# ZAX130/SmileCode

Measured on AMD Instinct MI355X. Metric: volume-pairs/sec (160x192x160) fwd+bwd, higher is better.
Workload: dtype f32; 1 GPU; ModeT 160x192x160 fp32, batch=1/GPU, full train step NCC+Grad3d fwd+bwd+Adam-amsgrad; global_batch=1, parallelism=dp1, allreduce=one flat all-reduce after backward

## Files before the change

### smilecode_amd/csrc/na.hip

```cpp
#include "common.h"
#include "drpb_reduce.h"
#include <cstdlib>

namespace {

constexpr int HD = 6;
constexpr int TZ = 4, TY = 4, TX = 16;
constexpr int HZ = TZ + 2, HY = TY + 2, HX = TX + 2;
constexpr int HVOX = HZ * HY * HX;
constexpr int NTHREADS = TZ * TY * TX;

struct TileGeom {
  int tiles_x, tiles_y, tiles_z;
};

__device__ __forceinline__ void tile_origin(int tile, const TileGeom g, int& z0, int& y0, int& x0) {
  const int tx = tile % g.tiles_x;
  const int t2 = tile / g.tiles_x;
  x0 = tx * TX;
  y0 = (t2 % g.tiles_y) * TY;
  z0 = (t2 / g.tiles_y) * TZ;
}

constexpr int KT_IT = (HVOX * 3 + NTHREADS - 1) / NTHREADS;
__device__ __forceinline__ float2 bf2_unpack(unsigned u) { return make_float2(__uint_as_float(u << 16), __uint_as_float(u & 0xffff0000u)); }
template <bool QK16 = false>
__device__ __forceinline__ void stage_k_load(float2 (&r)[KT_IT], const float* __restrict__ k, int64_t bbase, int z0, int y0,
                                             int x0, int D, int H, int W, int C, int hoff) {
  bool inside[KT_IT];
#pragma unroll
  for (int j = 0; j < KT_IT; ++j) {
    const int idx = min((int)threadIdx.x + j * NTHREADS, HVOX * 3 - 1);
    const int v = idx / 3, part = idx - v * 3;
    const int hx = v % HX, t = v / HX;
    const int hy = t % HY, hz = t / HY;
    const int z = z0 + hz - 1, y = y0 + hy - 1, x = x0 + hx - 1;
    const bool in = z >= 0 && z < D && y >= 0 && y < H && x >= 0 && x < W;
    const int64_t off = (bbase + (in ? ((int64_t)z * H + y) * W + x : 0)) * C + hoff + part * 2;
    if constexpr (QK16) r[j] = bf2_unpack(reinterpret_cast<const unsigned*>(k)[off >> 1]);
    else r[j] = *reinterpret_cast<const float2*>(k + off);
    inside[j] = in;
  }
#pragma unroll
  for (int j = 0; j < KT_IT; ++j) asm volatile("" : "+v"(r[j].x), "+v"(r[j].y));
#pragma unroll
  for (int j = 0; j < KT_IT; ++j)
    if (!inside[j]) r[j] = make_float2(0.f, 0.f);
}
__device__ __forceinline__ void stage_k_store(float* __restrict__ kt, const float2 (&r)[KT_IT]) {
#pragma unroll
  for (int j = 0; j < KT_IT; ++j) {
    const int idx = threadIdx.x + j * NTHREADS;
    if (idx < HVOX * 3) *reinterpret_cast<float2*>(kt + idx * 2) = r[j];
  }
}
template <bool QK16 = false>
__device__ __forceinline__ void stage_k_tile(float* __restrict__ kt, const float* __restrict__ k, int64_t bbase,
                                             int z0, int y0, int x0, int D, int H, int W, int C, int hoff) {
  float2 r[KT_IT];
  stage_k_load<QK16>(r, k, bbase, z0, y0, x0, D, H, W, C, hoff);
  stage_k_store(kt, r);
}

__device__ __forceinline__ void load6(const float* __restrict__ p, float (&r)[HD]) {
  const float2 a = *reinterpret_cast<const float2*>(p);
  const float2 b = *reinterpret_cast<const float2*>(p + 2);
  const float2 c = *reinterpret_cast<const float2*>(p + 4);
  r[0] = a.x; r[1] = a.y; r[2] = b.x; r[3] = b.y; r[4] = c.x; r[5] = c.y;
}

template <bool QK16>
__device__ __forceinline__ void load6g(const float* __restrict__ base, int64_t el, float (&r)[HD]) {
  if constexpr (QK16) {
    const unsigned* p = reinterpret_cast<const unsigned*>(base) + (el >> 1);
    const float2 a = bf2_unpack(p[0]), b = bf2_unpack(p[1]), c = bf2_unpack(p[2]);
    r[0] = a.x; r[1] = a.y; r[2] = b.x; r[3] = b.y; r[4] = c.x; r[5] = c.y;
  } else {
    load6(base + el, r);
  }
}

__device__ __forceinline__ void logits27(const float* __restrict__ kt, int lt, const float (&qs)[HD],
                                         const float* __restrict__ rpb_h, float (&lg)[27]) {
#pragma unroll
  for (int ki = 0; ki < 3; ++ki)
#pragma unroll
    for (int kj = 0; kj < 3; ++kj)
#pragma unroll
      for (int kk = 0; kk < 3; ++kk) {
        const int t = ki * 9 + kj * 3 + kk;
        float kv[HD];
        load6(kt + (lt + (ki * HY + kj) * HX + kk) * HD, kv);
        float s = rpb_h[t];
#pragma unroll
        for (int c = 0; c < HD; ++c) s = fmaf(qs[c], kv[c], s);
        lg[t] = s;
      }
}

__device__ __forceinline__ float softmax27(float (&lg)[27], float& m) {
  m = lg[0];
#pragma unroll
  for (int t = 1; t < 27; ++t) m = fmaxf(m, lg[t]);
  float s = 0.f;
#pragma unroll
  for (int t = 0; t < 27; ++t) {
    lg[t] = __expf(lg[t] - m);
    s += lg[t];
  }
  return 1.f / s;
}

template <bool QK16>
__global__ __launch_bounds__(NTHREADS) void na_fwd_kernel(const float* __restrict__ q, const float* __restrict__ k,
                                                          const float* __restrict__ rpb, float* __restrict__ out,
                                                          float* __restrict__ lse, int D, int H, int W, int heads,
                                                          float scale, TileGeom g) {
  __shared__ __attribute__((aligned(16))) float kt[HVOX * HD];
  __shared__ float rp[27];
  const int h = blockIdx.y, b = blockIdx.z;
  const int C = heads * HD;
  const int64_t V = (int64_t)D * H * W;
  int z0, y0, x0;
  tile_origin(blockIdx.x, g, z0, y0, x0);
  if (threadIdx.x < 27) rp[threadIdx.x] = rpb[h * 27 + threadIdx.x];
  stage_k_tile<QK16>(kt, k, (int64_t)b * V, z0, y0, x0, D, H, W, C, h * HD);
  __syncthreads();

  const int tx = threadIdx.x % TX, ty = (threadIdx.x / TX) % TY, tz = threadIdx.x / (TX * TY);
  const int z = z0 + tz, y = y0 + ty, x = x0 + tx;
  if (z >= D || y >= H || x >= W) return;
  const int64_t n = (int64_t)b * V + ((int64_t)z * H + y) * W + x;
  float qs[HD];
  load6g<QK16>(q, n * C + h * HD, qs);
#pragma unroll
  for (int c = 0; c < HD; ++c) qs[c] *= scale;
  float p[27];
  logits27(kt, (tz * HY + ty) * HX + tx, qs, rp, p);
  float mx;
  const float inv = softmax27(p, mx);
  if (lse) lse[n * heads + h] = mx - __logf(inv);
  float o0 = 0.f, o1 = 0.f, o2 = 0.f;
#pragma unroll
  for (int ki = 0; ki < 3; ++ki)
#pragma unroll
    for (int kj = 0; kj < 3; ++kj)
#pragma unroll
      for (int kk = 0; kk < 3; ++kk) {
        const float pv = p[ki * 9 + kj * 3 + kk];
        o0 += pv * (float)(ki - 1);
        o1 += pv * (float)(kj - 1);
        o2 += pv * (float)(kk - 1);
      }
  float* o = out + n * (heads * 3) + h * 3;
  o[0] = o0 * inv; o[1] = o1 * inv; o[2] = o2 * inv;
}

template <int N>
__device__ __forceinline__ void rs_step(float (&v)[32], int lane) {
  const bool up = (lane & N) != 0;
#pragma unroll
  for (int i = 0; i < N / 2; ++i) {
    const float keep = up ? v[i + N / 2] : v[i];
    const float send = up ? v[i] : v[i + N / 2];
    v[i] = keep + __shfl_xor(send, N, 64);
  }
}
__device__ __forceinline__ float wave_reduce_scatter32(const float (&v27)[27], int lane) {
  float v[32];
#pragma unroll
  for (int i = 0; i < 32; ++i) v[i] = i < 27 ? v27[i] : 0.f;
  rs_step<32>(v, lane); rs_step<16>(v, lane); rs_step<8>(v, lane); rs_step<4>(v, lane); rs_step<2>(v, lane);
  return v[0] + __shfl_xor(v[0], 1, 64);
}

constexpr int AUX = 5;

template <bool QK16>
__global__ __launch_bounds__(NTHREADS) void na_bwd_kernel(const float* __restrict__ q, const float* __restrict__ k,
                                                          const float* __restrict__ rpb, const float* __restrict__ out,
                                                          const float* __restrict__ lse, const float* __restrict__ dout,
                                                          float* __restrict__ dq, float* __restrict__ dk,
                                                          float* __restrict__ drpb_part, int D, int H, int W, int heads,
                                                          float scale, TileGeom g) {
  __shared__ __attribute__((aligned(16))) float kt[HVOX * HD];
  __shared__ __attribute__((aligned(16))) float qt[HVOX * HD];
  __shared__ float ax[HVOX * AUX];
  __shared__ float red[27 * (NTHREADS / 64)];
  __shared__ float rp[27];
  const int h = blockIdx.y, b = blockIdx.z;
  const int C = heads * HD;
  const int64_t V = (int64_t)D * H * W;
  int z0, y0, x0;
  tile_origin(blockIdx.x, g, z0, y0, x0);
  if (threadIdx.x < 27) rp[threadIdx.x] = rpb[h * 27 + threadIdx.x];
#ifdef NA_BWD_LDS_PAD
  __shared__ float lds_pad[NA_BWD_LDS_PAD];
  if (g.tiles_x < 0) { lds_pad[threadIdx.x % NA_BWD_LDS_PAD] = scale; __syncthreads(); rp[0] += lds_pad[(threadIdx.x * 7 + 1) % NA_BWD_LDS_PAD]; }
#endif
#ifdef NA_BWD_VGPR_CLOBBER
#define NA_STR2(x) #x
#define NA_STR(x) NA_STR2(x)
  asm volatile("" ::: "v" NA_STR(NA_BWD_VGPR_CLOBBER));
#endif
  {
    constexpr int AX_IT = (HVOX + NTHREADS - 1) / NTHREADS;
    float2 rk[KT_IT], rq[KT_IT];
    float ra[AX_IT][7];
    bool ain[AX_IT];
    stage_k_load<QK16>(rk, k, (int64_t)b * V, z0, y0, x0, D, H, W, C, h * HD);
    stage_k_load<QK16>(rq, q, (int64_t)b * V, z0, y0, x0, D, H, W, C, h * HD);
#pragma unroll
    for (int j = 0; j < AX_IT; ++j) {
      const int v = min((int)threadIdx.x + j * NTHREADS, HVOX - 1);
      const int hx = v % HX, t = v / HX;
      const int hy = t % HY, hz = t / HY;
      const int z = z0 + hz - 1, y = y0 + hy - 1, x = x0 + hx - 1;
      const bool in = z >= 0 && z < D && y >= 0 && y < H && x >= 0 && x < W;
      const int64_t n = (int64_t)b * V + (in ? ((int64_t)z * H + y) * W + x : 0);
      const float* go = dout + n * (heads * 3) + h * 3;
      const float* oo = out + n * (heads * 3) + h * 3;
      ra[j][0] = go[0]; ra[j][1] = go[1]; ra[j][2] = go[2];
      ra[j][3] = oo[0]; ra[j][4] = oo[1]; ra[j][5] = oo[2];
      ra[j][6] = lse[n * heads + h];
      ain[j] = in;
    }
#pragma unroll
    for (int j = 0; j < AX_IT; ++j)
#pragma unroll
      for (int e = 0; e < 7; ++e) asm volatile("" : "+v"(ra[j][e]));
#pragma unroll
    for (int j = 0; j < AX_IT; ++j)
      if (!ain[j]) {
#pragma unroll
        for (int e = 0; e < 7; ++e) ra[j][e] = 0.f;
      }
    stage_k_store(kt, rk);
    stage_k_store(qt, rq);
// ... 31 lines not shown
    for (int c = 0; c < HD; ++c) dqa[c] = 0.f;
#pragma unroll
    for (int ki = 0; ki < 3; ++ki)
#pragma unroll
      for (int kj = 0; kj < 3; ++kj)
#pragma unroll
        for (int kk = 0; kk < 3; ++kk) {
          const int t = ki * 9 + kj * 3 + kk;
          const float gt = (float)(ki - 1) * g0 + (float)(kj - 1) * g1 + (float)(kk - 1) * g2;
          const float d = __expf(dlv[t] - l) * (gt - u);
          dlv[t] = d;
          float kv[HD];
          load6(kt + (lt + (ki * HY + kj) * HX + kk) * HD, kv);
#pragma unroll
          for (int c = 0; c < HD; ++c) dqa[c] = fmaf(d, kv[c], dqa[c]);
        }
    float* dqp = dq + n * C + h * HD;
#pragma unroll
    for (int c = 0; c < HD; c += 2) *reinterpret_cast<float2*>(dqp + c) = make_float2(dqa[c] * scale, dqa[c + 1] * scale);
  }
  const int lane = threadIdx.x & 63, wv = threadIdx.x >> 6;
  {
    const float r = wave_reduce_scatter32(dlv, lane);
    if ((lane & 1) == 0 && (lane >> 1) < 27) red[wv * 27 + (lane >> 1)] = r;
  }
  if (live) {
    const int64_t n = (int64_t)b * V + ((int64_t)z * H + y) * W + x;
    const int lc = ((tz + 1) * HY + ty + 1) * HX + tx + 1;
    float kn[HD];
    load6(kt + lc * HD, kn);
#pragma unroll
    for (int c = 0; c < HD; ++c) kn[c] *= scale;
    float dka[HD];
#pragma unroll
    for (int c = 0; c < HD; ++c) dka[c] = 0.f;
#pragma unroll
    for (int ki = 0; ki < 3; ++ki)
#pragma unroll
      for (int kj = 0; kj < 3; ++kj)
#pragma unroll
        for (int kk = 0; kk < 3; ++kk) {
          const int lm = lc + ((1 - ki) * HY + (1 - kj)) * HX + (1 - kk);
          float qv[HD];
          load6(qt + lm * HD, qv);
          float lg = rp[ki * 9 + kj * 3 + kk];
#pragma unroll
          for (int c = 0; c < HD; ++c) lg = fmaf(qv[c], kn[c], lg);
          const float* am = ax + lm * AUX;
          const float gt = (float)(ki - 1) * am[0] + (float)(kj - 1) * am[1] + (float)(kk - 1) * am[2];
          const float d = __expf(lg - am[4]) * (gt - am[3]);
#pragma unroll
          for (int c = 0; c < HD; ++c) dka[c] = fmaf(d, qv[c], dka[c]);
        }
    float* dkp = dk + n * C + h * HD;
#pragma unroll
    for (int c = 0; c < HD; c += 2) *reinterpret_cast<float2*>(dkp + c) = make_float2(dka[c] * scale, dka[c + 1] * scale);
  }
  __syncthreads();
  if (threadIdx.x < 27) {
    float t = 0.f;
    for (int w = 0; w < NTHREADS / 64; ++w) t += red[w * 27 + threadIdx.x];
    const int64_t blk = ((int64_t)b * gridDim.y + h) * gridDim.x + blockIdx.x;
    drpb_part[blk * 27 + threadIdx.x] = t;
  }
}

constexpr int MY = 8, MX = 32, MHY = MY + 2, MHX = MX + 2, MHV = MHY * MHX;
constexpr int MSLOT = MHV * (2 * HD + AUX);
using NaBuf = __amdgpu_buffer_rsrc_t;
constexpr unsigned NA_OOB = 0x80000000u;
__device__ __forceinline__ NaBuf na_rsrc(const float* base, unsigned bytes) {
  const uint64_t a = reinterpret_cast<uint64_t>(base);
  const uint64_t u = ((uint64_t)(unsigned)__builtin_amdgcn_readfirstlane((unsigned)(a >> 32)) << 32) |
                     (uint64_t)(unsigned)__builtin_amdgcn_readfirstlane((unsigned)a);
  return __builtin_amdgcn_make_buffer_rsrc(reinterpret_cast<void*>(u), 0, (int)__builtin_amdgcn_readfirstlane(bytes), 0x00020000);
}
struct NaMarchArgs {
  const float* q; const float* k; const float* rpb; const float* out; const float* lse; const float* dout;
  float* dq; float* dk; float* drpb_part;
  int D, H, W, heads, tiles_x, tiles_y, nchunk, ZC;
  float scale;
};

template <bool QK16>
__global__ __launch_bounds__(NTHREADS, 2) void na_bwd_march_kernel(const NaMarchArgs a) {
  __shared__ __attribute__((aligned(16))) float ring[3 * MSLOT];
  __shared__ float red[27 * (NTHREADS / 64)];
  constexpr float LOG2E = 1.4426950408889634f;
  const int h = blockIdx.y, b = blockIdx.z;
  const int D = a.D, H = a.H, W = a.W, heads = a.heads;
  const int C = heads * HD, C3 = heads * 3;
  int t = blockIdx.x;
  const int x0 = (t % a.tiles_x) * MX; t /= a.tiles_x;
  const int y0 = (t % a.tiles_y) * MY;
  const int zs = (t / a.tiles_y) * a.ZC;
  const int ze = zs + a.ZC < D ? zs + a.ZC : D;
  float rp[27];
#pragma unroll
  for (int i = 0; i < 27; ++i) rp[i] = a.rpb[h * 27 + i];
  const int64_t V = (int64_t)D * H * W, HW = (int64_t)H * W;
  constexpr int QSZ = QK16 ? 2 : 4;
  const float* qb = reinterpret_cast<const float*>(reinterpret_cast<const char*>(a.q) + ((int64_t)b * V * C + h * HD) * QSZ);
  const float* kb = reinterpret_cast<const float*>(reinterpret_cast<const char*>(a.k) + ((int64_t)b * V * C + h * HD) * QSZ);
  const float* gb = a.dout + (int64_t)b * V * C3 + h * 3;
  const float* ob = a.out + (int64_t)b * V * C3 + h * 3;
  const float* lb = a.lse + (int64_t)b * V * heads + h;
  const unsigned qbytes = (unsigned)(HW * C * QSZ), gbytes = (unsigned)(HW * C3 * 4), lbytes = (unsigned)(HW * heads * 4);
  const float qmul = a.scale * LOG2E;

  constexpr int NIT = (MHV + NTHREADS - 1) / NTHREADS;
  unsigned oq[NIT], og[NIT], ol[NIT];
  int sl_[NIT];
#pragma unroll
  for (int j = 0; j < NIT; ++j) {
    const int v = threadIdx.x + j * NTHREADS;
    const bool on = v < MHV;
    const int hy = on ? v / MHX : 0, hx = on ? v - hy * MHX : 0;
    const int y = y0 + hy - 1, x = x0 + hx - 1;
    const bool ok = on && y >= 0 && y < H && x >= 0 && x < W;
    const unsigned n = (unsigned)(y * W + x);
    oq[j] = ok ? n * (unsigned)(C * QSZ) : NA_OOB;
    og[j] = ok ? n * (unsigned)(C3 * 4) : NA_OOB;
    ol[j] = ok ? n * (unsigned)(heads * 4) : NA_OOB;
    sl_[j] = on ? v : -1;
  }
  float2 rk[NIT][3], rq[NIT][3];
  float rg[NIT][3], ro[NIT][3], rl[NIT];
  auto load_plane = [&](int z) {
    const bool live = z >= 0 && z < D;
    const int64_t zo = live ? z : 0;
    const NaBuf bq = na_rsrc(reinterpret_cast<const float*>(reinterpret_cast<const char*>(qb) + zo * HW * C * QSZ), live ? qbytes : 0u);
    const NaBuf bk = na_rsrc(reinterpret_cast<const float*>(reinterpret_cast<const char*>(kb) + zo * HW * C * QSZ), live ? qbytes : 0u);
    const NaBuf bg = na_rsrc(gb + zo * HW * C3, live ? gbytes : 0u), bo = na_rsrc(ob + zo * HW * C3, live ? gbytes : 0u);
    const NaBuf bl = na_rsrc(lb + zo * HW * heads, live ? lbytes : 0u);
#pragma unroll
    for (int j = 0; j < NIT; ++j) {
#pragma unroll
      for (int c = 0; c < 3; ++c) {
        if constexpr (QK16) {
          rk[j][c] = bf2_unpack(__builtin_amdgcn_raw_buffer_load_b32(bk, (int)(oq[j] + c * 4), 0, 0));
          rq[j][c] = bf2_unpack(__builtin_amdgcn_raw_buffer_load_b32(bq, (int)(oq[j] + c * 4), 0, 0));
        } else {
          rk[j][c] = __builtin_bit_cast(float2, __builtin_amdgcn_raw_buffer_load_b64(bk, (int)(oq[j] + c * 8), 0, 0));
          rq[j][c] = __builtin_bit_cast(float2, __builtin_amdgcn_raw_buffer_load_b64(bq, (int)(oq[j] + c * 8), 0, 0));
        }
        rg[j][c] = __builtin_bit_cast(float, __builtin_amdgcn_raw_buffer_load_b32(bg, (int)(og[j] + c * 4), 0, 0));
        ro[j][c] = __builtin_bit_cast(float, __builtin_amdgcn_raw_buffer_load_b32(bo, (int)(og[j] + c * 4), 0, 0));
      }
      rl[j] = __builtin_bit_cast(float, __builtin_amdgcn_raw_buffer_load_b32(bl, (int)ol[j], 0, 0));
    }
  };
  auto store_plane = [&](int slot) {
    float* kt = ring + slot * MSLOT;
    float* qt = kt + MHV * HD;
    float* gu = qt + MHV * HD;
    float* ls = gu + MHV * 4;
#pragma unroll
    for (int j = 0; j < NIT; ++j) {
      if (sl_[j] < 0) continue;
      const int v = sl_[j];
#pragma unroll
      for (int c = 0; c < 3; ++c) {
        *reinterpret_cast<float2*>(kt + v * HD + c * 2) = rk[j][c];
        *reinterpret_cast<float2*>(qt + v * HD + c * 2) = make_float2(rq[j][c].x * qmul, rq[j][c].y * qmul);
      }
      *reinterpret_cast<float4*>(gu + v * 4) =
          make_float4(rg[j][0], rg[j][1], rg[j][2], rg[j][0] * ro[j][0] + rg[j][1] * ro[j][1] + rg[j][2] * ro[j][2]);
      ls[v] = rl[j] * LOG2E;
    }
  };

  const int tx = threadIdx.x % MX, ty = threadIdx.x / MX;
  const int y = y0 + ty, x = x0 + tx;
  const bool live = y < H && x < W;
  const int hc = (ty + 1) * MHX + tx + 1;
  float dlv[27];
#pragma unroll
  for (int i = 0; i < 27; ++i) dlv[i] = 0.f;

  load_plane(zs - 1); store_plane(0);
  load_plane(zs); store_plane(1);
  load_plane(zs + 1); store_plane(2);
  load_plane(zs + 2);
  __syncthreads();
  for (int z = zs, i = 0; z < ze; ++z, ++i) {
    const int s0 = i % 3, s1 = (i + 1) % 3, s2 = (i + 2) % 3;
    if (live) {
      const int sof[3] = {s0 * MSLOT, s1 * MSLOT, s2 * MSLOT};
      const float* kc = ring + sof[1];
      const int64_t n = (int64_t)b * V + ((int64_t)z * H + y) * W + x;
      float qs[HD], dqa[HD];
      load6(kc + MHV * HD + hc * HD, qs);
#pragma unroll
      for (int c = 0; c < HD; ++c) dqa[c] = 0.f;
      const float4 gc = *reinterpret_cast<const float4*>(kc + 2 * MHV * HD + hc * 4);
      const float l = kc[2 * MHV * HD + MHV * 4 + hc];
#pragma unroll
      for (int ki = 0; ki < 3; ++ki) {
        const float* kt = ring + sof[ki];
#pragma unroll
        for (int kj = 0; kj < 3; ++kj)
#pragma unroll
          for (int kk = 0; kk < 3; ++kk) {
            const int tt = ki * 9 + kj * 3 + kk;
            float kv[HD];
            load6(kt + (hc + (kj - 1) * MHX + (kk - 1)) * HD, kv);
            float lg = fmaf(rp[tt], LOG2E, -l);
#pragma unroll
            for (int c = 0; c < HD; ++c) lg = fmaf(qs[c], kv[c], lg);
            const float gt = (float)(ki - 1) * gc.x + (float)(kj - 1) * gc.y + (float)(kk - 1) * gc.z;
            const float d = __builtin_amdgcn_exp2f(lg) * (gt - gc.w);
            dlv[tt] += d;
#pragma unroll
            for (int c = 0; c < HD; ++c) dqa[c] = fmaf(d, kv[c], dqa[c]);
          }
      }
      float* dqp = a.dq + n * C + h * HD;
#pragma unroll
      for (int c = 0; c < HD; c += 2) *reinterpret_cast<float2*>(dqp + c) = make_float2(dqa[c] * a.scale, dqa[c + 1] * a.scale);
      float kn[HD], dka[HD];
      load6(kc + hc * HD, kn);
#pragma unroll
      for (int c = 0; c < HD; ++c) dka[c] = 0.f;
#pragma unroll
      for (int ki = 0; ki < 3; ++ki) {
        const float* qt = ring + sof[2 - ki] + MHV * HD;
        const float* gu = qt + MHV * HD;
        const float* ls = gu + MHV * 4;
#pragma unroll
        for (int kj = 0; kj < 3; ++kj)
#pragma unroll
          for (int kk = 0; kk < 3; ++kk) {
            const int lm = hc + (1 - kj) * MHX + (1 - kk);
            float qv[HD];
            load6(qt + lm * HD, qv);
            float lg = fmaf(rp[ki * 9 + kj * 3 + kk], LOG2E, -ls[lm]);
#pragma unroll
            for (int c = 0; c < HD; ++c) lg = fmaf(qv[c], kn[c], lg);
            const float4 gm = *reinterpret_cast<const float4*>(gu + lm * 4);
            const float gt = (float)(ki - 1) * gm.x + (float)(kj - 1) * gm.y + (float)(kk - 1) * gm.z;
            const float d = __builtin_amdgcn_exp2f(lg) * (gt - gm.w);
#pragma unroll
            for (int c = 0; c < HD; ++c) dka[c] = fmaf(d, qv[c], dka[c]);
          }
      }
      float* dkp = a.dk + n * C + h * HD;
      constexpr float ILOG2E = 0.6931471805599453f;
#pragma unroll
      for (int c = 0; c < HD; c += 2) *reinterpret_cast<float2*>(dkp + c) = make_float2(dka[c] * ILOG2E, dka[c + 1] * ILOG2E);
    }
    __syncthreads();
    store_plane(s0);
    __syncthreads();
    load_plane(z + 3);
  }
  const int lane = threadIdx.x & 63, wv = threadIdx.x >> 6;
  {
    const float r = wave_reduce_scatter32(dlv, lane);
    if ((lane & 1) == 0 && (lane >> 1) < 27) red[wv * 27 + (lane >> 1)] = r;
  }
  __syncthreads();
  if (threadIdx.x < 27) {
    float s = 0.f;
    for (int w = 0; w < NTHREADS / 64; ++w) s += red[w * 27 + threadIdx.x];
    const int64_t blk = ((int64_t)b * gridDim.y + h) * gridDim.x + blockIdx.x;
    a.drpb_part[blk * 27 + threadIdx.x] = s;
  }
}

struct NaMarchPlan { int tiles_x, tiles_y, nchunk, zc; bool on; };
inline NaMarchPlan na_march_plan(int B, int D, int H, int W, int heads, int hd) {
  NaMarchPlan p;
  p.tiles_x = cdiv(W, MX); p.tiles_y = cdiv(H, MY);
  p.on = hd == HD && (int64_t)D * H * W >= 1500000 && (int64_t)H * W * heads * HD * 4 < 0x7fffffffLL;
  const int cols = B * heads * p.tiles_x * p.tiles_y;
  int want = 2000;
#ifdef MODET_TUNING
  if (const char* e = getenv("MODET_NA_WGS")) want = atoi(e);
  if (const char* e = getenv("MODET_NA_MARCH")) p.on = p.on && e[0] != '0';
#endif
  int best = (want + cols - 1) / cols;
  const int maxn = D / 8 > 0 ? D / 8 : 1;
  best = best < 1 ? 1 : (best > maxn ? maxn : best);
  p.zc = cdiv(D, best);
  p.nchunk = cdiv(D, p.zc);
  return p;
}

constexpr int GC = 8;

__device__ __forceinline__ void stage_chunk(float* __restrict__ dst, const float* __restrict__ srcp, int64_t bbase, int z0,
                                            int y0, int x0, int D, int H, int W, int C, int coff) {
  for (int idx = threadIdx.x; idx < HVOX * 2; idx += NTHREADS) {
    const int v = idx >> 1, part = idx & 1;
    const int hx = v % HX, t = v / HX;
    const int hy = t % HY, hz = t / HY;
    const int z = z0 + hz - 1, y = y0 + hy - 1, x = x0 + hx - 1;
    float4 val = make_float4(0.f, 0.f, 0.f, 0.f);
    if (z >= 0 && z < D && y >= 0 && y < H && x >= 0 && x < W)
      val = *reinterpret_cast<const float4*>(srcp + (bbase + ((int64_t)z * H + y) * W + x) * C + coff + part * 4);
    *reinterpret_cast<float4*>(dst + v * GC + part * 4) = val;
  }
}
__device__ __forceinline__ void load8(const float* __restrict__ p, float (&r)[GC]) {
  const float4 a = *reinterpret_cast<const float4*>(p), b = *reinterpret_cast<const float4*>(p + 4);
  r[0] = a.x; r[1] = a.y; r[2] = a.z; r[3] = a.w; r[4] = b.x; r[5] = b.y; r[6] = b.z; r[7] = b.w;
}
__device__ __forceinline__ float dot8(const float (&a)[GC], const float (&b)[GC]) {
  float s = 0.f;
#pragma unroll
  for (int c = 0; c < GC; ++c) s = fmaf(a[c], b[c], s);
  return s;
}

__global__ __launch_bounds__(NTHREADS) void na_fwd_gen_kernel(const float* __restrict__ q, const float* __restrict__ k,
                                                              const float* __restrict__ rpb, float* __restrict__ out,
                                                              float* __restrict__ lse, int D, int H, int W, int heads,
                                                              int hd, float scale, TileGeom g) {
  __shared__ __attribute__((aligned(16))) float kt[HVOX * GC];
  __shared__ float rp[27];
  const int h = blockIdx.y, b = blockIdx.z;
  const int C = heads * hd;
  const int64_t V = (int64_t)D * H * W;
  int z0, y0, x0;
  tile_origin(blockIdx.x, g, z0, y0, x0);
  if (threadIdx.x < 27) rp[threadIdx.x] = rpb[h * 27 + threadIdx.x];
  const int tx = threadIdx.x % TX, ty = (threadIdx.x / TX) % TY, tz = threadIdx.x / (TX * TY);
  const int z = z0 + tz, y = y0 + ty, x = x0 + tx;
  const bool live = z < D && y < H && x < W;
  const int64_t n = (int64_t)b * V + ((int64_t)(live ? z : 0) * H + (live ? y : 0)) * W + (live ? x : 0);
  const int lt = (tz * HY + ty) * HX + tx;
  float p[27];
#pragma unroll
  for (int t = 0; t < 27; ++t) p[t] = 0.f;
  for (int c0 = 0; c0 < hd; c0 += GC) {
    __syncthreads();
    stage_chunk(kt, k, (int64_t)b * V, z0, y0, x0, D, H, W, C, h * hd + c0);
    __syncthreads();
    if (live) {
      float qs[GC];
      load8(q + n * C + h * hd + c0, qs);
#pragma unroll
      for (int ki = 0; ki < 3; ++ki)
#pragma unroll
        for (int kj = 0; kj < 3; ++kj)
#pragma unroll
          for (int kk = 0; kk < 3; ++kk) {
            float kv[GC];
            load8(kt + (lt + (ki * HY + kj) * HX + kk) * GC, kv);
// ... 76 lines not shown
#pragma unroll
      for (int ki = 0; ki < 3; ++ki)
#pragma unroll
        for (int kj = 0; kj < 3; ++kj)
#pragma unroll
          for (int kk = 0; kk < 3; ++kk) {
            const int t = ki * 9 + kj * 3 + kk;
            float v8[GC];
            load8(kt + (lt + (ki * HY + kj) * HX + kk) * GC, v8);
            dlq[t] += dot8(qn, v8);
            load8(qt + (lc + ((1 - ki) * HY + (1 - kj)) * HX + (1 - kk)) * GC, v8);
            dlk[t] += dot8(v8, kn);
          }
    }
  }
  if (live) {
    const float* ac = ax + lc * AUX;
    const float g0 = ac[0], g1 = ac[1], g2 = ac[2], u = ac[3], l = ac[4];
#pragma unroll
    for (int ki = 0; ki < 3; ++ki)
#pragma unroll
      for (int kj = 0; kj < 3; ++kj)
#pragma unroll
        for (int kk = 0; kk < 3; ++kk) {
          const int t = ki * 9 + kj * 3 + kk;
          const float gt = (float)(ki - 1) * g0 + (float)(kj - 1) * g1 + (float)(kk - 1) * g2;
          dlq[t] = __expf(fmaf(dlq[t], scale, rp[t]) - l) * (gt - u);
          const float* am = ax + (lc + ((1 - ki) * HY + (1 - kj)) * HX + (1 - kk)) * AUX;
          const float gm = (float)(ki - 1) * am[0] + (float)(kj - 1) * am[1] + (float)(kk - 1) * am[2];
          dlk[t] = __expf(fmaf(dlk[t], scale, rp[t]) - am[4]) * (gm - am[3]);
        }
  }
  const int lane = threadIdx.x & 63, wv = threadIdx.x >> 6;
  {
    const float r = wave_reduce_scatter32(dlq, lane);
    if ((lane & 1) == 0 && (lane >> 1) < 27) red[wv * 27 + (lane >> 1)] = r;
  }
  const int64_t n = (int64_t)b * V + ((int64_t)(live ? z : 0) * H + (live ? y : 0)) * W + (live ? x : 0);
  for (int c0 = 0; c0 < hd; c0 += GC) {
    __syncthreads();
    stage_chunk(kt, k, (int64_t)b * V, z0, y0, x0, D, H, W, C, h * hd + c0);
    stage_chunk(qt, q, (int64_t)b * V, z0, y0, x0, D, H, W, C, h * hd + c0);
    __syncthreads();
    if (live) {
      float dqa[GC], dka[GC];
#pragma unroll
      for (int c = 0; c < GC; ++c) { dqa[c] = 0.f; dka[c] = 0.f; }
#pragma unroll
      for (int ki = 0; ki < 3; ++ki)
#pragma unroll
        for (int kj = 0; kj < 3; ++kj)
#pragma unroll
          for (int kk = 0; kk < 3; ++kk) {
            const int t = ki * 9 + kj * 3 + kk;
            float v8[GC];
            load8(kt + (lt + (ki * HY + kj) * HX + kk) * GC, v8);
#pragma unroll
            for (int c = 0; c < GC; ++c) dqa[c] = fmaf(dlq[t], v8[c], dqa[c]);
            load8(qt + (lc + ((1 - ki) * HY + (1 - kj)) * HX + (1 - kk)) * GC, v8);
#pragma unroll
            for (int c = 0; c < GC; ++c) dka[c] = fmaf(dlk[t], v8[c], dka[c]);
          }
      float* dqp = dq + n * C + h * hd + c0;
      float* dkp = dk + n * C + h * hd + c0;
      *reinterpret_cast<float4*>(dqp) = make_float4(dqa[0] * scale, dqa[1] * scale, dqa[2] * scale, dqa[3] * scale);
      *reinterpret_cast<float4*>(dqp + 4) = make_float4(dqa[4] * scale, dqa[5] * scale, dqa[6] * scale, dqa[7] * scale);
      *reinterpret_cast<float4*>(dkp) = make_float4(dka[0] * scale, dka[1] * scale, dka[2] * scale, dka[3] * scale);
      *reinterpret_cast<float4*>(dkp + 4) = make_float4(dka[4] * scale, dka[5] * scale, dka[6] * scale, dka[7] * scale);
    }
  }
  __syncthreads();
  if (threadIdx.x < 27) {
    float t = 0.f;
    for (int w = 0; w < NTHREADS / 64; ++w) t += red[w * 27 + threadIdx.x];
    const int64_t blk = ((int64_t)b * gridDim.y + h) * gridDim.x + blockIdx.x;
    drpb_part[blk * 27 + threadIdx.x] = t;
  }
}

inline bool gen_hd_ok(int hd) { return hd >= GC && hd <= 128 && hd % GC == 0; }

inline TileGeom geom(int D, int H, int W) { return TileGeom{cdiv(W, TX), cdiv(H, TY), cdiv(D, TZ)}; }

}

extern "C" {

int modet_na_fwd_t(const void* q, const void* k, int qk_bf16, const float* rpb, float* out, float* lse, int B, int D, int H, int W,
                   int heads, int hd, float scale, modet_stream_t stream) {
  if (!qk_bf16) return modet_na_fwd((const float*)q, (const float*)k, rpb, out, lse, B, D, H, W, heads, hd, scale, stream);
  MODET_CHECK_PTR(q); MODET_CHECK_PTR(k); MODET_CHECK_PTR(rpb); MODET_CHECK_PTR(out);
  MODET_CHECK_DIM(B > 0 && D > 0 && H > 0 && W > 0 && heads > 0);
  if (hd != HD) return MODET_ERR_UNSUPPORTED;
  const TileGeom g = geom(D, H, W);
  dim3 grid(g.tiles_x * g.tiles_y * g.tiles_z, heads, B);
  hipLaunchKernelGGL(na_fwd_kernel<true>, grid, dim3(NTHREADS), 0, (hipStream_t)stream, (const float*)q, (const float*)k, rpb, out,
                     lse, D, H, W, heads, scale, g);
  return modet_launch_status();
}

int modet_na_fwd(const float* q, const float* k, const float* rpb, float* out, float* lse, int B, int D, int H, int W,
                 int heads, int hd, float scale, modet_stream_t stream) {
  MODET_CHECK_PTR(q); MODET_CHECK_PTR(k); MODET_CHECK_PTR(rpb); MODET_CHECK_PTR(out);
  MODET_CHECK_DIM(B > 0 && D > 0 && H > 0 && W > 0 && heads > 0);
  if (hd != HD && !gen_hd_ok(hd)) return MODET_ERR_UNSUPPORTED;
  const TileGeom g = geom(D, H, W);
  dim3 grid(g.tiles_x * g.tiles_y * g.tiles_z, heads, B);
  if (hd == HD)
    hipLaunchKernelGGL(na_fwd_kernel<false>, grid, dim3(NTHREADS), 0, (hipStream_t)stream, q, k, rpb, out, lse, D, H, W, heads,
                       scale, g);
  else
    hipLaunchKernelGGL(na_fwd_gen_kernel, grid, dim3(NTHREADS), 0, (hipStream_t)stream, q, k, rpb, out, lse, D, H, W,
                       heads, hd, scale, g);
  return modet_launch_status();
}

size_t modet_na_bwd_ws_bytes(int B, int D, int H, int W, int heads) {
  const TileGeom g = geom(D, H, W);
  size_t fl = (size_t)B * heads * g.tiles_x * g.tiles_y * g.tiles_z * 27;
  fl += fl & 1;
  return fl * sizeof(float) + drpb_scratch_bytes(B, heads);
}

int modet_na_bwd_t(const void* qv, const void* kv, int qk_bf16, const float* rpb, const float* out, const float* lse,
                   const float* d_out, float* d_q, float* d_k, float* d_rpb, void* ws, size_t ws_bytes, int B, int D,
                   int H, int W, int heads, int hd, float scale, modet_stream_t stream) {
  const float* q = (const float*)qv;
  const float* k = (const float*)kv;
  MODET_CHECK_PTR(q); MODET_CHECK_PTR(k); MODET_CHECK_PTR(rpb); MODET_CHECK_PTR(out); MODET_CHECK_PTR(lse);
  MODET_CHECK_PTR(d_out); MODET_CHECK_PTR(d_q); MODET_CHECK_PTR(d_k); MODET_CHECK_PTR(ws);
  MODET_CHECK_DIM(B > 0 && D > 0 && H > 0 && W > 0 && heads > 0);
  if (hd != HD && (qk_bf16 || !gen_hd_ok(hd))) return MODET_ERR_UNSUPPORTED;
  if (ws_bytes < modet_na_bwd_ws_bytes(B, D, H, W, heads)) return MODET_ERR_WORKSPACE;
  hipStream_t s = (hipStream_t)stream;
  const NaMarchPlan mp = na_march_plan(B, D, H, W, heads, hd);
  if (mp.on) {
    const int64_t nblk = (int64_t)mp.tiles_x * mp.tiles_y * mp.nchunk;
    NaMarchArgs a{q, k, rpb, out, lse, d_out, d_q, d_k, (float*)ws, D, H, W, heads, mp.tiles_x, mp.tiles_y, mp.nchunk, mp.zc, scale};
    if (qk_bf16) hipLaunchKernelGGL(na_bwd_march_kernel<true>, dim3((unsigned)nblk, heads, B), dim3(NTHREADS), 0, s, a);
    else hipLaunchKernelGGL(na_bwd_march_kernel<false>, dim3((unsigned)nblk, heads, B), dim3(NTHREADS), 0, s, a);
    size_t fl = (size_t)B * heads * nblk * 27;
    fl += fl & 1;
    if (d_rpb) drpb_reduce((float*)ws, ws, fl * sizeof(float), d_rpb, B, heads, nblk, s);
    return modet_launch_status();
  }
  const TileGeom g = geom(D, H, W);
  const int64_t nblk = (int64_t)g.tiles_x * g.tiles_y * g.tiles_z;
  float* part = (float*)ws;
  dim3 grid((unsigned)nblk, heads, B);
  if (hd == HD) {
    if (qk_bf16) hipLaunchKernelGGL(na_bwd_kernel<true>, grid, dim3(NTHREADS), 0, s, q, k, rpb, out, lse, d_out, d_q, d_k, part, D, H, W,
                                    heads, scale, g);
    else hipLaunchKernelGGL(na_bwd_kernel<false>, grid, dim3(NTHREADS), 0, s, q, k, rpb, out, lse, d_out, d_q, d_k, part, D, H, W,
                            heads, scale, g);
  } else {
    hipLaunchKernelGGL(na_bwd_gen_kernel, grid, dim3(NTHREADS), 0, s, q, k, rpb, out, lse, d_out, d_q, d_k, part, D, H, W,
                       heads, hd, scale, g);
  }
  size_t fl = (size_t)B * heads * nblk * 27;
  fl += fl & 1;
  if (d_rpb) drpb_reduce(part, ws, fl * sizeof(float), d_rpb, B, heads, nblk, s);
  return modet_launch_status();
}

int64_t modet_na_bwd_partial_rows(int B, int D, int H, int W, int heads, int hd) {
  if (B <= 0 || D <= 0 || H <= 0 || W <= 0 || heads <= 0) return 0;
  const NaMarchPlan mp = na_march_plan(B, D, H, W, heads, hd);
  if (mp.on) return (int64_t)mp.tiles_x * mp.tiles_y * mp.nchunk;
  const TileGeom g = geom(D, H, W);
  return (int64_t)g.tiles_x * g.tiles_y * g.tiles_z;
}

int modet_na_bwd(const float* q, const float* k, const float* rpb, const float* out, const float* lse,
                 const float* d_out, float* d_q, float* d_k, float* d_rpb, void* ws, size_t ws_bytes, int B, int D,
                 int H, int W, int heads, int hd, float scale, modet_stream_t stream) {
  return modet_na_bwd_t(q, k, 0, rpb, out, lse, d_out, d_q, d_k, d_rpb, ws, ws_bytes, B, D, H, W, heads, hd, scale, stream);
}

}
```

Measured before the change: 140.0 volume-pairs/sec.

## Split NA backward march into dq/dk thread roles and add z-marching forward kernel

The backward march kernel now launches twice as many threads. Half of them compute dq and the other half compute dk for the same voxel, instead of one thread doing both serially, which shortens each thread's dependency chain. A new forward kernel marches along z with a three-plane ring of K tiles in shared memory, replacing the per-tile halo restaging of the old forward kernel. The bf16 staging registers now hold packed values and unpack at store time to save registers. The costs are larger workgroups, launch-bound changes that may constrain registers, and a prologue fma-ordering trick for the gu term.

After: 140.9 volume-pairs/sec (median of 6 runs). About the same (+0.6%).

```diff
diff --git a/smilecode_amd/csrc/na.hip b/smilecode_amd/csrc/na.hip
--- a/smilecode_amd/csrc/na.hip
+++ b/smilecode_amd/csrc/na.hip
@@ -1,6 +1,7 @@
 #include "common.h"
 #include "drpb_reduce.h"
 #include <cstdlib>
+#include <type_traits>
 
 namespace {
 
@@ -24,6 +25,9 @@
 
 constexpr int KT_IT = (HVOX * 3 + NTHREADS - 1) / NTHREADS;
 __device__ __forceinline__ float2 bf2_unpack(unsigned u) { return make_float2(__uint_as_float(u << 16), __uint_as_float(u & 0xffff0000u)); }
+template <bool QK16> using StgPair = typename std::conditional<QK16, unsigned, float2>::type;
+__device__ __forceinline__ float2 stg_f2(unsigned u) { return bf2_unpack(u); }
+__device__ __forceinline__ float2 stg_f2(float2 v) { return v; }
 template <bool QK16 = false>
 __device__ __forceinline__ void stage_k_load(float2 (&r)[KT_IT], const float* __restrict__ k, int64_t bbase, int z0, int y0,
                                              int x0, int D, int H, int W, int C, int hoff) {
@@ -80,22 +84,29 @@
   }
 }
 
-__device__ __forceinline__ void logits27(const float* __restrict__ kt, int lt, const float (&qs)[HD],
-                                         const float* __restrict__ rpb_h, float (&lg)[27]) {
-#pragma unroll
-  for (int ki = 0; ki < 3; ++ki)
+template <int SX>
+__device__ __forceinline__ void logits27_planes(const float* __restrict__ kt, const int (&pz)[3], int lt,
+                                                const float (&qs)[HD], const float* __restrict__ rpb_h, float (&lg)[27]) {
+#pragma unroll
+  for (int ki = 0; ki < 3; ++ki) {
 #pragma unroll
     for (int kj = 0; kj < 3; ++kj)
 #pragma unroll
       for (int kk = 0; kk < 3; ++kk) {
         const int t = ki * 9 + kj * 3 + kk;
         float kv[HD];
-        load6(kt + (lt + (ki * HY + kj) * HX + kk) * HD, kv);
+        load6(kt + (lt + pz[ki] + kj * SX + kk) * HD, kv);
         float s = rpb_h[t];
 #pragma unroll
         for (int c = 0; c < HD; ++c) s = fmaf(qs[c], kv[c], s);
         lg[t] = s;
       }
+  }
+}
+__device__ __forceinline__ void logits27(const float* __restrict__ kt, int lt, const float (&qs)[HD],
+                                         const float* __restrict__ rpb_h, float (&lg)[27]) {
+  constexpr int pz[3] = {0, HY * HX, 2 * HY * HX};
+  logits27_planes<HX>(kt, pz, lt, qs, rpb_h, lg);
 }
 
 __device__ __forceinline__ float softmax27(float (&lg)[27], float& m) {
@@ -109,6 +120,25 @@
     s += lg[t];
   }
   return 1.f / s;
+}
+
+__device__ __forceinline__ void na_fwd_voxel(float (&p)[27], float* __restrict__ o, float* __restrict__ lse, int64_t li) {
+  float mx;
+  const float inv = softmax27(p, mx);
+  if (lse) lse[li] = mx - __logf(inv);
+  float o0 = 0.f, o1 = 0.f, o2 = 0.f;
+#pragma unroll
+  for (int ki = 0; ki < 3; ++ki)
+#pragma unroll
+    for (int kj = 0; kj < 3; ++kj)
+#pragma unroll
+      for (int kk = 0; kk < 3; ++kk) {
+        const float pv = p[ki * 9 + kj * 3 + kk];
+        o0 += pv * (float)(ki - 1);
+        o1 += pv * (float)(kj - 1);
+        o2 += pv * (float)(kk - 1);
+      }
+  o[0] = o0 * inv; o[1] = o1 * inv; o[2] = o2 * inv;
 }
 
 template <bool QK16>
@@ -137,23 +167,7 @@
   for (int c = 0; c < HD; ++c) qs[c] *= scale;
   float p[27];
   logits27(kt, (tz * HY + ty) * HX + tx, qs, rp, p);
-  float mx;
-  const float inv = softmax27(p, mx);
-  if (lse) lse[n * heads + h] = mx - __logf(inv);
-  float o0 = 0.f, o1 = 0.f, o2 = 0.f;
-#pragma unroll
-  for (int ki = 0; ki < 3; ++ki)
-#pragma unroll
-    for (int kj = 0; kj < 3; ++kj)
-#pragma unroll
-      for (int kk = 0; kk < 3; ++kk) {
-        const float pv = p[ki * 9 + kj * 3 + kk];
-        o0 += pv * (float)(ki - 1);
-        o1 += pv * (float)(kj - 1);
-        o2 += pv * (float)(kk - 1);
-      }
-  float* o = out + n * (heads * 3) + h * 3;
-  o[0] = o0 * inv; o[1] = o1 * inv; o[2] = o2 * inv;
+  na_fwd_voxel(p, out + n * (heads * 3) + h * 3, lse, n * heads + h);
 }
 
 template <int N>
@@ -351,8 +365,11 @@
   float scale;
 };
 
+constexpr int MTHREADS = 2 * NTHREADS;
+static_assert(2 * (3 * MSLOT + 27 * (NTHREADS / 64)) * sizeof(float) <= 160 * 1024, "two workgroups (ring + red) per CU");
+
 template <bool QK16>
-__global__ __launch_bounds__(NTHREADS, 2) void na_bwd_march_kernel(const NaMarchArgs a) {
+__global__ __launch_bounds__(MTHREADS, 4) void na_bwd_march_kernel(const NaMarchArgs a) {
   __shared__ __attribute__((aligned(16))) float ring[3 * MSLOT];
   __shared__ float red[27 * (NTHREADS / 64)];
   constexpr float LOG2E = 1.4426950408889634f;
@@ -377,12 +394,12 @@
   const unsigned qbytes = (unsigned)(HW * C * QSZ), gbytes = (unsigned)(HW * C3 * 4), lbytes = (unsigned)(HW * heads * 4);
   const float qmul = a.scale * LOG2E;
 
-  constexpr int NIT = (MHV + NTHREADS - 1) / NTHREADS;
+  constexpr int NIT = (MHV + MTHREADS - 1) / MTHREADS;
   unsigned oq[NIT], og[NIT], ol[NIT];
   int sl_[NIT];
 #pragma unroll
   for (int j = 0; j < NIT; ++j) {
-    const int v = threadIdx.x + j * NTHREADS;
+    const int v = threadIdx.x + j * MTHREADS;
     const bool on = v < MHV;
     const int hy = on ? v / MHX : 0, hx = on ? v - hy * MHX : 0;
     const int y = y0 + hy - 1, x = x0 + hx - 1;
@@ -393,7 +410,7 @@
     ol[j] = ok ? n * (unsigned)(heads * 4) : NA_OOB;
     sl_[j] = on ? v : -1;
   }
-  float2 rk[NIT][3], rq[NIT][3];
+  StgPair<QK16> rk[NIT][3], rq[NIT][3];
   float rg[NIT][3], ro[NIT][3], rl[NIT];
   auto load_plane = [&](int z) {
     const bool live = z >= 0 && z < D;
@@ -407,8 +424,8 @@
 #pragma unroll
       for (int c = 0; c < 3; ++c) {
         if constexpr (QK16) {
-          rk[j][c] = bf2_unpack(__builtin_amdgcn_raw_buffer_load_b32(bk, (int)(oq[j] + c * 4), 0, 0));
-          rq[j][c] = bf2_unpack(__builtin_amdgcn_raw_buffer_load_b32(bq, (int)(oq[j] + c * 4), 0, 0));
+          rk[j][c] = __builtin_amdgcn_raw_buffer_load_b32(bk, (int)(oq[j] + c * 4), 0, 0);
+          rq[j][c] = __builtin_amdgcn_raw_buffer_load_b32(bq, (int)(oq[j] + c * 4), 0, 0);
         } else {
           rk[j][c] = __builtin_bit_cast(float2, __builtin_amdgcn_raw_buffer_load_b64(bk, (int)(oq[j] + c * 8), 0, 0));
           rq[j][c] = __builtin_bit_cast(float2, __builtin_amdgcn_raw_buffer_load_b64(bq, (int)(oq[j] + c * 8), 0, 0));
@@ -419,7 +436,7 @@
       rl[j] = __builtin_bit_cast(float, __builtin_amdgcn_raw_buffer_load_b32(bl, (int)ol[j], 0, 0));
     }
   };
-  auto store_plane = [&](int slot) {
+  auto store_plane = [&](int slot, bool prologue) {
     float* kt = ring + slot * MSLOT;
     float* qt = kt + MHV * HD;
     float* gu = qt + MHV * HD;
@@ -430,16 +447,20 @@
       const int v = sl_[j];
 #pragma unroll
       for (int c = 0; c < 3; ++c) {
-        *reinterpret_cast<float2*>(kt + v * HD + c * 2) = rk[j][c];
-        *reinterpret_cast<float2*>(qt + v * HD + c * 2) = make_float2(rq[j][c].x * qmul, rq[j][c].y * qmul);
+        const float2 qv = stg_f2(rq[j][c]);
+        *reinterpret_cast<float2*>(kt + v * HD + c * 2) = stg_f2(rk[j][c]);
+        *reinterpret_cast<float2*>(qt + v * HD + c * 2) = make_float2(qv.x * qmul, qv.y * qmul);
       }
+      const float uz = fmaf(rg[j][1], ro[j][1], rg[j][0] * ro[j][0]), uy = fmaf(rg[j][0], ro[j][0], rg[j][1] * ro[j][1]);
       *reinterpret_cast<float4*>(gu + v * 4) =
-          make_float4(rg[j][0], rg[j][1], rg[j][2], rg[j][0] * ro[j][0] + rg[j][1] * ro[j][1] + rg[j][2] * ro[j][2]);
+          make_float4(rg[j][0], rg[j][1], rg[j][2], fmaf(rg[j][2], ro[j][2], prologue && v >= NTHREADS ? uy : uz));
       ls[v] = rl[j] * LOG2E;
     }
   };
 
-  const int tx = threadIdx.x % MX, ty = threadIdx.x / MX;
+  const bool qrole = threadIdx.x < NTHREADS;
+  const int vt = threadIdx.x % NTHREADS;
+  const int tx = vt % MX, ty = vt / MX;
   const int y = y0 + ty, x = x0 + tx;
   const bool live = y < H && x < W;
   const int hc = (ty + 1) * MHX + tx + 1;
@@ -447,9 +468,9 @@
 #pragma unroll
   for (int i = 0; i < 27; ++i) dlv[i] = 0.f;
 
-  load_plane(zs - 1); store_plane(0);
-  load_plane(zs); store_plane(1);
-  load_plane(zs + 1); store_plane(2);
+  load_plane(zs - 1); store_plane(0, true);
+  load_plane(zs); store_plane(1, true);
+  load_plane(zs + 1); store_plane(2, true);
   load_plane(zs + 2);
   __syncthreads();
   for (int z = zs, i = 0; z < ze; ++z, ++i) {
@@ -458,73 +479,76 @@
       const int sof[3] = {s0 * MSLOT, s1 * MSLOT, s2 * MSLOT};
       const float* kc = ring + sof[1];
       const int64_t n = (int64_t)b * V + ((int64_t)z * H + y) * W + x;
-      float qs[HD], dqa[HD];
-      load6(kc + MHV * HD + hc * HD, qs);
-#pragma unroll
-      for (int c = 0; c < HD; ++c) dqa[c] = 0.f;
-      const float4 gc = *reinterpret_cast<const float4*>(kc + 2 * MHV * HD + hc * 4);
-      const float l = kc[2 * MHV * HD + MHV * 4 + hc];
-#pragma unroll
-      for (int ki = 0; ki < 3; ++ki) {
-        const float* kt = ring + sof[ki];
-#pragma unroll
-        for (int kj = 0; kj < 3; ++kj)
-#pragma unroll
-          for (int kk = 0; kk < 3; ++kk) {
-            const int tt = ki * 9 + kj * 3 + kk;
-            float kv[HD];
-            load6(kt + (hc + (kj - 1) * MHX + (kk - 1)) * HD, kv);
-            float lg = fmaf(rp[tt], LOG2E, -l);
-#pragma unroll
-            for (int c = 0; c < HD; ++c) lg = fmaf(qs[c], kv[c], lg);
-            const float gt = (float)(ki - 1) * gc.x + (float)(kj - 1) * gc.y + (float)(kk - 1) * gc.z;
-            const float d = __builtin_amdgcn_exp2f(lg) * (gt - gc.w);
-            dlv[tt] += d;
-#pragma unroll
-            for (int c = 0; c < HD; ++c) dqa[c] = fmaf(d, kv[c], dqa[c]);
-          }
+      constexpr float ILOG2E = 0.6931471805599453f;
+      float* dqp = a.dq + n * C + h * HD;
+      float* dkp = a.dk + n * C + h * HD;
+      if (qrole) {
+        float qs[HD], dqa[HD];
+        load6(kc + MHV * HD + hc * HD, qs);
+#pragma unroll
+        for (int c = 0; c < HD; ++c) dqa[c] = 0.f;
+        const float4 gc = *reinterpret_cast<const float4*>(kc + 2 * MHV * HD + hc * 4);
+        const float l = kc[2 * MHV * HD + MHV * 4 + hc];
+#pragma unroll
+        for (int ki = 0; ki < 3; ++ki) {
+          const float* kt = ring + sof[ki];
+#pragma unroll
+          for (int kj = 0; kj < 3; ++kj)
+#pragma unroll
+            for (int kk = 0; kk < 3; ++kk) {
+              const int tt = ki * 9 + kj * 3 + kk;
+              float kv[HD];
+              load6(kt + (hc + (kj - 1) * MHX + (kk - 1)) * HD, kv);
+              float lg = fmaf(rp[tt], LOG2E, -l);
+#pragma unroll
+              for (int c = 0; c < HD; ++c) lg = fmaf(qs[c], kv[c], lg);
+              const float gt = (float)(ki - 1) * gc.x + (float)(kj - 1) * gc.y + (float)(kk - 1) * gc.z;
+              const float d = __builtin_amdgcn_exp2f(lg) * (gt - gc.w);
+              dlv[tt] += d;
+#pragma unroll
+              for (int c = 0; c < HD; ++c) dqa[c] = fmaf(d, kv[c], dqa[c]);
+            }
+        }
+#pragma unroll
+        for (int c = 0; c < HD; c += 2) *reinterpret_cast<float2*>(dqp + c) = make_float2(dqa[c] * a.scale, dqa[c + 1] * a.scale);
+      } else {
+        float kn[HD], dka[HD];
+        load6(kc + hc * HD, kn);
+#pragma unroll
+        for (int c = 0; c < HD; ++c) dka[c] = 0.f;
+#pragma unroll
+        for (int ki = 0; ki < 3; ++ki) {
+          const float* qt = ring + sof[2 - ki] + MHV * HD;
+          const float* gu = qt + MHV * HD;
+          const float* ls = gu + MHV * 4;
+#pragma unroll
+          for (int kj = 0; kj < 3; ++kj)
+#pragma unroll
+            for (int kk = 0; kk < 3; ++kk) {
+              const int lm = hc + (1 - kj) * MHX + (1 - kk);
+              float qv[HD];
+              load6(qt + lm * HD, qv);
+              float lg = fmaf(rp[ki * 9 + kj * 3 + kk], LOG2E, -ls[lm]);
+#pragma unroll
+              for (int c = 0; c < HD; ++c) lg = fmaf(qv[c], kn[c], lg);
+              const float4 gm = *reinterpret_cast<const float4*>(gu + lm * 4);
+              const float gt = (float)(ki - 1) * gm.x + (float)(kj - 1) * gm.y + (float)(kk - 1) * gm.z;
+              const float d = __builtin_amdgcn_exp2f(lg) * (gt - gm.w);
+#pragma unroll
+              for (int c = 0; c < HD; ++c) dka[c] = fmaf(d, qv[c], dka[c]);
+            }
+        }
+#pragma unroll
+        for (int c = 0; c < HD; c += 2) *reinterpret_cast<float2*>(dkp + c) = make_float2(dka[c] * ILOG2E, dka[c + 1] * ILOG2E);
       }
-      float* dqp = a.dq + n * C + h * HD;
-#pragma unroll
-      for (int c = 0; c < HD; c += 2) *reinterpret_cast<float2*>(dqp + c) = make_float2(dqa[c] * a.scale, dqa[c + 1] * a.scale);
-      float kn[HD], dka[HD];
-      load6(kc + hc * HD, kn);
-#pragma unroll
-      for (int c = 0; c < HD; ++c) dka[c] = 0.f;
-#pragma unroll
-      for (int ki = 0; ki < 3; ++ki) {
-        const float* qt = ring + sof[2 - ki] + MHV * HD;
-        const float* gu = qt + MHV * HD;
-        const float* ls = gu + MHV * 4;
-#pragma unroll
-        for (int kj = 0; kj < 3; ++kj)
-#pragma unroll
-          for (int kk = 0; kk < 3; ++kk) {
-            const int lm = hc + (1 - kj) * MHX + (1 - kk);
-            float qv[HD];
-            load6(qt + lm * HD, qv);
-            float lg = fmaf(rp[ki * 9 + kj * 3 + kk], LOG2E, -ls[lm]);
-#pragma unroll
-            for (int c = 0; c < HD; ++c) lg = fmaf(qv[c], kn[c], lg);
-            const float4 gm = *reinterpret_cast<const float4*>(gu + lm * 4);
-            const float gt = (float)(ki - 1) * gm.x + (float)(kj - 1) * gm.y + (float)(kk - 1) * gm.z;
-            const float d = __builtin_amdgcn_exp2f(lg) * (gt - gm.w);
-#pragma unroll
-            for (int c = 0; c < HD; ++c) dka[c] = fmaf(d, qv[c], dka[c]);
-          }
-      }
-      float* dkp = a.dk + n * C + h * HD;
-      constexpr float ILOG2E = 0.6931471805599453f;
-#pragma unroll
-      for (int c = 0; c < HD; c += 2) *reinterpret_cast<float2*>(dkp + c) = make_float2(dka[c] * ILOG2E, dka[c + 1] * ILOG2E);
     }
     __syncthreads();
-    store_plane(s0);
+    store_plane(s0, false);
     __syncthreads();
     load_plane(z + 3);
   }
   const int lane = threadIdx.x & 63, wv = threadIdx.x >> 6;
-  {
+  if (qrole) {
     const float r = wave_reduce_scatter32(dlv, lane);
     if ((lane & 1) == 0 && (lane >> 1) < 27) red[wv * 27 + (lane >> 1)] = r;
   }
@@ -534,6 +558,105 @@
     for (int w = 0; w < NTHREADS / 64; ++w) s += red[w * 27 + threadIdx.x];
     const int64_t blk = ((int64_t)b * gridDim.y + h) * gridDim.x + blockIdx.x;
     a.drpb_part[blk * 27 + threadIdx.x] = s;
+  }
+}
+
+struct NaFwdMarchArgs {
+  const float* q; const float* k; const float* rpb; float* out; float* lse;
+  int D, H, W, heads, tiles_x, tiles_y, ZC;
+  float scale;
+};
+
+template <bool QK16>
+__global__ __launch_bounds__(NTHREADS, 6) void na_fwd_march_kernel(const NaFwdMarchArgs a) {
+  constexpr int KSLOT = MHV * HD;
+  __shared__ __attribute__((aligned(16))) float ring[3 * KSLOT];
+  const int h = blockIdx.y, b = blockIdx.z;
+  const int D = a.D, H = a.H, W = a.W, heads = a.heads;
+  const int C = heads * HD;
+  int t = blockIdx.x;
+  const int x0 = (t % a.tiles_x) * MX; t /= a.tiles_x;
+  const int y0 = (t % a.tiles_y) * MY;
+  const int zs = (t / a.tiles_y) * a.ZC;
+  const int ze = zs + a.ZC < D ? zs + a.ZC : D;
+  float rp[27];
+#pragma unroll
+  for (int i = 0; i < 27; ++i) rp[i] = a.rpb[h * 27 + i];
+  const int64_t V = (int64_t)D * H * W, HW = (int64_t)H * W;
+  constexpr int QSZ = QK16 ? 2 : 4;
+  const char* qb = reinterpret_cast<const char*>(a.q) + ((int64_t)b * V * C + h * HD) * QSZ;
+  const char* kb = reinterpret_cast<const char*>(a.k) + ((int64_t)b * V * C + h * HD) * QSZ;
+  const unsigned qbytes = (unsigned)(HW * C * QSZ);
+
+  constexpr int NIT = (MHV + NTHREADS - 1) / NTHREADS;
+  unsigned ok_[NIT];
+  int sl_[NIT];
+#pragma unroll
+  for (int j = 0; j < NIT; ++j) {
+    const int v = threadIdx.x + j * NTHREADS;
+    const bool on = v < MHV;
+    const int hy = on ? v / MHX : 0, hx = on ? v - hy * MHX : 0;
+    const int y = y0 + hy - 1, x = x0 + hx - 1;
+    const bool ok = on && y >= 0 && y < H && x >= 0 && x < W;
+    ok_[j] = ok ? (unsigned)(y * W + x) * (unsigned)(C * QSZ) : NA_OOB;
+    sl_[j] = on ? v : -1;
+  }
+  const int tx = threadIdx.x % MX, ty = threadIdx.x / MX;
+  const int y = y0 + ty, x = x0 + tx;
+  const bool live = y < H && x < W;
+  const unsigned oqc = live ? (unsigned)(y * W + x) * (unsigned)(C * QSZ) : NA_OOB;
+  const int lt = ty * MHX + tx;
+
+  float2 rk[NIT][3], rq[3];
+  auto plane_rsrc = [&](const char* base, int z) {
+    const bool in = z >= 0 && z < D;
+    return na_rsrc(reinterpret_cast<const float*>(base + (int64_t)(in ? z : 0) * HW * C * QSZ), in ? qbytes : 0u);
+  };
+  auto load3 = [&](float2 (&r)[3], const NaBuf bf, unsigned off) {
+#pragma unroll
+    for (int c = 0; c < 3; ++c) {
+      if constexpr (QK16) r[c] = bf2_unpack(__builtin_amdgcn_raw_buffer_load_b32(bf, (int)(off + c * 4), 0, 0));
+      else r[c] = __builtin_bit_cast(float2, __builtin_amdgcn_raw_buffer_load_b64(bf, (int)(off + c * 8), 0, 0));
+    }
+  };
+  auto load_plane = [&](int z) {
+    const NaBuf bk = plane_rsrc(kb, z);
+#pragma unroll
+    for (int j = 0; j < NIT; ++j) load3(rk[j], bk, ok_[j]);
+  };
+  auto store_plane = [&](int slot) {
+    float* kt = ring + slot * KSLOT;
+#pragma unroll
+    for (int j = 0; j < NIT; ++j) {
+      if (sl_[j] < 0) continue;
+#pragma unroll
+      for (int c = 0; c < 3; ++c) *reinterpret_cast<float2*>(kt + sl_[j] * HD + c * 2) = rk[j][c];
+    }
+  };
+
+  load3(rq, plane_rsrc(qb, zs), oqc);
+  load_plane(zs - 1); store_plane(0);
+  load_plane(zs); store_plane(1);
+  load_plane(zs + 1); store_plane(2);
+  load_plane(zs + 2);
+  __syncthreads();
+  for (int z = zs, i = 0; z < ze; ++z, ++i) {
+    const int s0 = i % 3, s1 = (i + 1) % 3, s2 = (i + 2) % 3;
+    float qs[HD] = {rq[0].x, rq[0].y, rq[1].x, rq[1].y, rq[2].x, rq[2].y};
+    load3(rq, plane_rsrc(qb, z + 1), oqc);
+    if (live) {
+      const int64_t n = (int64_t)b * V + ((int64_t)z * H + y) * W + x;
+#pragma unroll
+      for (int c = 0; c < HD; ++c) qs[c] *= a.scale;
+      float p[27];
+      const int pz[3] = {s0 * MHV, s1 * MHV, s2 * MHV};
+      logits27_planes<MHX>(ring, pz, lt, qs, rp, p);
+      na_fwd_voxel(p, a.out + n * (heads * 3) + h * 3, a.lse, n * heads + h);
+    }
+    __syncthreads();
+    store_plane(s0);
+    __syncthreads();
+    load_plane(z + 3);
   }
 }
 
@@ -776,6 +899,21 @@
 
 inline TileGeom geom(int D, int H, int W) { return TileGeom{cdiv(W, TX), cdiv(H, TY), cdiv(D, TZ)}; }
 
+template <bool QK16>
+void na_fwd_launch(const float* q, const float* k, const float* rpb, float* out, float* lse, int B, int D, int H, int W,
+                   int heads, float scale, hipStream_t s) {
+  const NaMarchPlan mp = na_march_plan(B, D, H, W, heads, HD);
+  if (mp.on) {
+    const NaFwdMarchArgs a{q, k, rpb, out, lse, D, H, W, heads, mp.tiles_x, mp.tiles_y, mp.zc, scale};
+    hipLaunchKernelGGL(na_fwd_march_kernel<QK16>, dim3((unsigned)(mp.tiles_x * mp.tiles_y * mp.nchunk), heads, B),
+                       dim3(NTHREADS), 0, s, a);
+    return;
+  }
+  const TileGeom g = geom(D, H, W);
+  hipLaunchKernelGGL(na_fwd_kernel<QK16>, dim3(g.tiles_x * g.tiles_y * g.tiles_z, heads, B), dim3(NTHREADS), 0, s, q, k, rpb,
+                     out, lse, D, H, W, heads, scale, g);
+}
+
 }
 
 extern "C" {
@@ -786,10 +924,7 @@
   MODET_CHECK_PTR(q); MODET_CHECK_PTR(k); MODET_CHECK_PTR(rpb); MODET_CHECK_PTR(out);
   MODET_CHECK_DIM(B > 0 && D > 0 && H > 0 && W > 0 && heads > 0);
   if (hd != HD) return MODET_ERR_UNSUPPORTED;
-  const TileGeom g = geom(D, H, W);
-  dim3 grid(g.tiles_x * g.tiles_y * g.tiles_z, heads, B);
-  hipLaunchKernelGGL(na_fwd_kernel<true>, grid, dim3(NTHREADS), 0, (hipStream_t)stream, (const float*)q, (const float*)k, rpb, out,
-                     lse, D, H, W, heads, scale, g);
+  na_fwd_launch<true>((const float*)q, (const float*)k, rpb, out, lse, B, D, H, W, heads, scale, (hipStream_t)stream);
   return modet_launch_status();
 }
 
@@ -798,14 +933,13 @@
   MODET_CHECK_PTR(q); MODET_CHECK_PTR(k); MODET_CHECK_PTR(rpb); MODET_CHECK_PTR(out);
   MODET_CHECK_DIM(B > 0 && D > 0 && H > 0 && W > 0 && heads > 0);
   if (hd != HD && !gen_hd_ok(hd)) return MODET_ERR_UNSUPPORTED;
-  const TileGeom g = geom(D, H, W);
-  dim3 grid(g.tiles_x * g.tiles_y * g.tiles_z, heads, B);
-  if (hd == HD)
-    hipLaunchKernelGGL(na_fwd_kernel<false>, grid, dim3(NTHREADS), 0, (hipStream_t)stream, q, k, rpb, out, lse, D, H, W, heads,
-                       scale, g);
-  else
-    hipLaunchKernelGGL(na_fwd_gen_kernel, grid, dim3(NTHREADS), 0, (hipStream_t)stream, q, k, rpb, out, lse, D, H, W,
-                       heads, hd, scale, g);
+  if (hd == HD) {
+    na_fwd_launch<false>(q, k, rpb, out, lse, B, D, H, W, heads, scale, (hipStream_t)stream);
+  } else {
+    const TileGeom g = geom(D, H, W);
+    hipLaunchKernelGGL(na_fwd_gen_kernel, dim3(g.tiles_x * g.tiles_y * g.tiles_z, heads, B), dim3(NTHREADS), 0,
+                       (hipStream_t)stream, q, k, rpb, out, lse, D, H, W, heads, hd, scale, g);
+  }
   return modet_launch_status();
 }
 
@@ -831,8 +965,8 @@
   if (mp.on) {
     const int64_t nblk = (int64_t)mp.tiles_x * mp.tiles_y * mp.nchunk;
     NaMarchArgs a{q, k, rpb, out, lse, d_out, d_q, d_k, (float*)ws, D, H, W, heads, mp.tiles_x, mp.tiles_y, mp.nchunk, mp.zc, scale};
-    if (qk_bf16) hipLaunchKernelGGL(na_bwd_march_kernel<true>, dim3((unsigned)nblk, heads, B), dim3(NTHREADS), 0, s, a);
-    else hipLaunchKernelGGL(na_bwd_march_kernel<false>, dim3((unsigned)nblk, heads, B), dim3(NTHREADS), 0, s, a);
+    if (qk_bf16) hipLaunchKernelGGL(na_bwd_march_kernel<true>, dim3((unsigned)nblk, heads, B), dim3(MTHREADS), 0, s, a);
+    else hipLaunchKernelGGL(na_bwd_march_kernel<false>, dim3((unsigned)nblk, heads, B), dim3(MTHREADS), 0, s, a);
     size_t fl = (size_t)B * heads * nblk * 27;
     fl += fl & 1;
     if (d_rpb) drpb_reduce((float*)ws, ws, fl * sizeof(float), d_rpb, B, heads, nblk, s);
```
